# InternRobotics/InternNav

Measured on NVIDIA H100. Metric: InternVLA-N1 policy-steps/sec (batch RGB-D+text->action), higher is better.
Workload: dtype bf16

## Files before the change

### internnav_b200/csrc/attention_cache_wgmma.cu

```cuda
#include <math.h>

#include <mutex>

#include "dec_tile.cuh"

namespace n1 {
namespace {

constexpr int HD = 128, BKEY = 64, kStages = 4;
constexpr int kHalf = BKEY * 128;
constexpr int kBlockBytes = 2 * kHalf;
constexpr int kStageBytes = 2 * kBlockBytes;
constexpr int kQBytes = 2 * 128 * 128;
constexpr int kConsumerWarps = 8;
constexpr int kThreads = 32 * kConsumerWarps + 32;
constexpr int kSmem = kStages * kStageBytes + kQBytes + 256 + 1024;
static_assert(kSmem <= 232448, "attention_cache: shared memory budget");

struct CacheArgs {
  const bf16 *k, *v;
  int ldkv;
  bf16* o;
  int ldo;
  const int *cu_q, *ctx, *row0;
// ... 114 lines not shown
      const int k0 = n * BKEY + quad * 2;
      float alpha[2], m_s[2];
#pragma unroll
      for (int h = 0; h < 2; ++h) {
        float m = mx[h];
#pragma unroll
        for (int j = 0; j < 8; ++j)
#pragma unroll
          for (int e = 0; e < 2; ++e)
            if (k0 + j * 8 + e < vis[h]) m = fmaxf(m, s[4 * j + 2 * h + e]);
        m = fmaxf(m, __shfl_xor_sync(0xffffffffu, m, 1));
        m = fmaxf(m, __shfl_xor_sync(0xffffffffu, m, 2));
        alpha[h] = fast_exp2((mx[h] - m) * a.scale_log2);
        mx[h] = m;
        m_s[h] = m * a.scale_log2;
        sum[h] *= alpha[h];
      }
#pragma unroll
      for (int j = 0; j < 16; ++j) {
        o[4 * j + 0] *= alpha[0], o[4 * j + 1] *= alpha[0];
        o[4 * j + 2] *= alpha[1], o[4 * j + 3] *= alpha[1];
      }
      uint32_t pa[4][4];
#pragma unroll
      for (int j = 0; j < 8; ++j)
#pragma unroll
        for (int h = 0; h < 2; ++h) {
          const int kk = k0 + j * 8;
          const float p0 = kk < vis[h] ? fast_exp2(s[4 * j + 2 * h] * a.scale_log2 - m_s[h]) : 0.f;
          const float p1 = kk + 1 < vis[h] ? fast_exp2(s[4 * j + 2 * h + 1] * a.scale_log2 - m_s[h]) : 0.f;
          sum[h] += p0 + p1;
          pa[j >> 1][(j & 1) * 2 + h] = pack_bf16(p0, p1);
        }
      wgmma_fence();
#pragma unroll
      for (int ks = 0; ks < 4; ++ks) {
        const uint64_t bd = wgmma_desc_sw128(smem_u32(sV + ks * 16 * 128), kHalf);
        wgmma_rs<1>(o, pa[ks], bd, 1u);
      }
      wgmma_commit();
      wgmma_wait<0>();
      __syncwarp();
      if (lane == 0) mbar_arrive(empty + st);
    }
#pragma unroll
    for (int h = 0; h < 2; ++h) {
      float l = sum[h];
      l += __shfl_xor_sync(0xffffffffu, l, 1);
      l += __shfl_xor_sync(0xffffffffu, l, 2);
      const float inv = l > 0.f ? 1.0f / l : 0.f;
      if (qrow[h] >= 0) {
        const int m = m_a + h * 8;
        bf16* orow = a.o + (long)(q_start + qrow[h]) * a.ldo + (kh * G + m % G) * HD + quad * 2;
#pragma unroll
        for (int j = 0; j < 16; ++j)
          *reinterpret_cast<uint32_t*>(orow + j * 8) = pack_bf16(o[4 * j + 2 * h] * inv, o[4 * j + 2 * h + 1] * inv);
      }
    }
  }
}

}

void attention_cache(const CacheAttnParams& p, cudaStream_t stream) {
  if (p.batch <= 0) return;
  N1_CHECK(p.heads_kv > 0 && p.heads_q % p.heads_kv == 0 && p.heads_q / p.heads_kv <= 64,
           "attention_cache: heads_q must be a multiple of heads_kv (at most 64 per group)");
  N1_CHECK(p.ldq % 8 == 0 && p.ldkv % 8 == 0 && p.ldo % 8 == 0 && p.max_chunk > 0 && p.q_rows > 0 && p.kv_rows > 0,
           "attention_cache: bad strides / sizes");
  N1_CHECK((reinterpret_cast<uintptr_t>(p.k) & 15) == 0 && (reinterpret_cast<uintptr_t>(p.v) & 15) == 0 &&
               (reinterpret_cast<uintptr_t>(p.o) & 15) == 0,
           "attention_cache: 16-byte alignment");
  N1_CHECK(p.batch <= 65535 && p.heads_kv <= 65535, "attention_cache: grid too large");
  static std::once_flag once;
  std::call_once(once, [] { cudaFuncSetAttribute(attn_cache_kernel, cudaFuncAttributeMaxDynamicSharedMemorySize, kSmem); });
  CacheArgs a;
  a.k = p.k, a.v = p.v, a.ldkv = p.ldkv, a.o = p.o, a.ldo = p.ldo;
  a.cu_q = p.cu_q, a.ctx = p.ctx, a.row0 = p.row0;
  a.group = p.heads_q / p.heads_kv;
  a.rows_wg = 64 / a.group;
  a.scale_log2 = p.scale * 1.4426950408889634f;
  const long qd[3] = {HD, p.heads_q, p.q_rows}, qs[2] = {HD, p.ldq};
  const int qb[3] = {64, a.group, a.rows_wg};
  CUtensorMap tmQ = tma_map_3d_sw128(p.q, qd, qs, qb);
  CUtensorMap tmK = tma_map_2d(p.k, p.kv_rows, (long)p.heads_kv * HD, p.ldkv, BKEY, 64, true);
  CUtensorMap tmV = tma_map_2d(p.v, p.kv_rows, (long)p.heads_kv * HD, p.ldkv, BKEY, 64, true);
  const int tiles = (p.max_chunk + 2 * a.rows_wg - 1) / (2 * a.rows_wg);
  dim3 grid(tiles, p.heads_kv, p.batch);
  attn_cache_kernel<<<grid, kThreads, kSmem, stream>>>(tmQ, tmK, tmV, a);
  prof_count_launch();
  N1_CUDA(cudaGetLastError());
}

}
```

### internnav_b200/csrc/dec_attn_block.cu

```cuda
#include <mutex>

#include "dec_tile.cuh"

namespace n1 {
namespace {

constexpr int D = 384, HD = 48, BM = 64;
constexpr int kABytes = BM * D * 2;
constexpr int kSlots = 2, kSlotBytes = D * 64 * 2;
constexpr int kKvRow = 112;
constexpr int kKvBytes = BM * kKvRow;
constexpr int kConsumerWarps = 8;
constexpr int kThreads = 32 * kConsumerWarps + 128;
constexpr int kSmem = 2 * kABytes + kSlots * kSlotBytes + 2 * 2 * kKvBytes + 256 + 1024;
static_assert(kSmem <= 232448, "dec_attn_block: shared memory budget (227 KB per block)");

struct DecAttnArgs {
  bf16* x;
  int ldx;
  const float* ln_w;
  const float* ln_b;
  float eps;
  const float* b_in;
  const float* b_o;
  const bf16* kv;
  int ldkv;
  int mtok;
  int Ns, T, tpt, tiles_per_env, tiles;
  int causal;
};

__device__ __forceinline__ void warpgroup_barrier(int g) { asm volatile("bar.sync %0, 128;" ::"r"(2 + g) : "memory"); }

template <bool kSelf>
__global__ void __launch_bounds__(kThreads, 1)
dec_attn_kernel(const __grid_constant__ CUtensorMap tmIn, const __grid_constant__ CUtensorMap tmO, const DecAttnArgs args) {
  constexpr int NP = kSelf ? 3 * HD : HD;
  constexpr int kHeadBytes = NP * 64 * 2;
  extern __shared__ uint8_t smem_raw[];
  uint8_t* smem = reinterpret_cast<uint8_t*>((reinterpret_cast<uintptr_t>(smem_raw) + 1023) & ~uintptr_t(1023));
  uint8_t* sA = smem;
  uint8_t* sO = smem + kABytes;
  uint8_t* sW = sO + kABytes;
  uint8_t* sKV = sW + kSlots * kSlotBytes;
  uint64_t* bars = reinterpret_cast<uint64_t*>(sKV + 4 * kKvBytes);
  uint64_t* full = bars;
  uint64_t* empty = bars + kSlots;

  const int warp = threadIdx.x >> 5, lane = threadIdx.x & 31;
  if (threadIdx.x == 0) {
    tma_prefetch_desc(&tmIn), tma_prefetch_desc(&tmO);
    for (int s = 0; s < kSlots; ++s) mbar_init(&full[s], 1), mbar_init(&empty[s], kConsumerWarps);
    fence_mbar_init();
  }
  __syncthreads();

  if (warp >= kConsumerWarps) {
    setmaxnreg_dec<kProducerRegs>();
    if (warp == kConsumerWarps && lane == 0) {
      Ring<kSlots> r;
      for (int t = blockIdx.x; t < args.tiles; t += gridDim.x) {
        for (int hp = 0; hp < 4; ++hp)
          for (int kb = 0; kb < D / 64; ++kb) {
            mbar_wait(&empty[r.slot], r.phase ^ 1);
            mbar_arrive_expect_tx(&full[r.slot], 2 * kHeadBytes);
            uint8_t* dst = sW + r.slot * kSlotBytes;
#pragma unroll
            for (int g = 0; g < 2; ++g) {
              const int h = 4 * g + hp;
#pragma unroll
              for (int part = 0; part < NP / HD; ++part)
                tma_load_2d(dst + g * kHeadBytes + part * HD * 128, &tmIn, &full[r.slot], kb * 64, part * D + h * HD);
            }
            r.advance();
          }
        for (int kb = 0; kb < D / 64; ++kb) {
          mbar_wait(&empty[r.slot], r.phase ^ 1);
          mbar_arrive_expect_tx(&full[r.slot], kSlotBytes);
          uint8_t* dst = sW + r.slot * kSlotBytes;
          tma_load_2d(dst, &tmO, &full[r.slot], kb * 64, 0);
          tma_load_2d(dst + kSlotBytes / 2, &tmO, &full[r.slot], kb * 64, 192);
          r.advance();
        }
      }
    }
  } else {
    setmaxnreg_inc<kConsumerRegs>();
    const int cw = warp;
    const int g = cw >> 2;
    const int wtid = threadIdx.x & 127;
    const int quad = lane & 3;
    const int r0 = (cw & 3) * 16 + (lane >> 2);
    uint8_t* sK = sKV + g * 2 * kKvBytes;
    uint8_t* sV = sK + kKvBytes;
    const float sl2 = 0.14433756729740643f * 1.4426950408889634f;
    Ring<kSlots> ring;
    for (int t = blockIdx.x; t < args.tiles; t += gridDim.x) {
      const int env = t / args.tiles_per_env;
      const int traj0 = (t - env * args.tiles_per_env) * args.tpt;
      const int ntraj = min(args.tpt, args.Ns - traj0);
      const long row0 = ((long)env * args.Ns + traj0) * args.T;
      const int nrows = ntraj * args.T;
      consumer_barrier();
      ln384_to_tile<false>(sA, args.x, args.ldx, row0, nrows, args.ln_w, args.ln_b, args.eps, cw, lane);
      fence_proxy_async_smem();
      consumer_barrier();

      for (int hp = 0; hp < 4; ++hp) {
        const int h = 4 * g + hp;
        warpgroup_barrier(g);
        if (!kSelf) {
          const bf16* kb0 = args.kv + (long)env * args.mtok * args.ldkv + h * HD;
          for (int c = wtid; c < 2 * BM * 6; c += 128) {
            const int v = c / (BM * 6), j = (c / 6) % BM, ch = c % 6;
            uint4 val = make_uint4(0u, 0u, 0u, 0u);
            if (j < args.mtok) val = __ldg(reinterpret_cast<const uint4*>(kb0 + (long)j * args.ldkv + v * D + ch * 8));
            *reinterpret_cast<uint4*>((v ? sV : sK) + j * kKvRow + ch * 16) = val;
          }
        }
        float acc[NP / 2];
        mma_k384(acc, sA, sW, full, empty, ring, kSlotBytes, g * kHeadBytes, lane, [] {});
        uint32_t qf[3][4];
#pragma unroll
        for (int j = 0; j < NP / 8; ++j) {
          const int part = j / 6, c = (j % 6) * 8 + quad * 2;
          const float2 b = __ldg(reinterpret_cast<const float2*>(args.b_in + part * D + h * HD + c));
          const uint32_t lo = pack_bf16(acc[4 * j] + b.x, acc[4 * j + 1] + b.y);
          const uint32_t hi = pack_bf16(acc[4 * j + 2] + b.x, acc[4 * j + 3] + b.y);
          if (part == 0) {
            qf[j >> 1][(j & 1) * 2] = lo, qf[j >> 1][(j & 1) * 2 + 1] = hi;
          } else {
            uint8_t* buf = part == 1 ? sK : sV;
            *reinterpret_cast<uint32_t*>(buf + r0 * kKvRow + c * 2) = lo;
            *reinterpret_cast<uint32_t*>(buf + (r0 + 8) * kKvRow + c * 2) = hi;
          }
        }
        warpgroup_barrier(g);
        int lo_key[2], hi_key[2];
#pragma unroll
        for (int r = 0; r < 2; ++r) {
          const int qi = r0 + 8 * r;
          if (kSelf) {
            lo_key[r] = qi / args.T * args.T;
            hi_key[r] = args.causal ? qi : lo_key[r] + args.T - 1;
          } else {
            lo_key[r] = 0, hi_key[r] = args.mtok - 1;
          }
        }
        float o[6][4], inv0, inv1;
        attn_hd48_16rows<4>(qf, sK, sV, kKvRow, lo_key, hi_key, sl2, lane, o, inv0, inv1);
#pragma unroll
        for (int i = 0; i < 6; ++i) {
          const int col = h * HD + i * 8 + quad * 2;
          *reinterpret_cast<uint32_t*>(sO + sw128_offset(r0, col)) = pack_bf16(o[i][0] * inv0, o[i][1] * inv0);
          *reinterpret_cast<uint32_t*>(sO + sw128_offset(r0 + 8, col)) = pack_bf16(o[i][2] * inv1, o[i][3] * inv1);
        }
      }
      fence_proxy_async_smem();
      consumer_barrier();
      float y[96] = {};
      mma_k384(y, sO, sW, full, empty, ring, kSlotBytes, g * (kSlotBytes / 2), lane, [] {});
      residual_epilogue_192<false>(y, args.x, args.ldx, args.x, args.ldx, args.b_o, row0, nrows, g, r0, quad);
    }
  }
}

template <bool kSelf>
void launch_dec_attn(const bf16* w_in, const bf16* w_o, const DecAttnArgs& a, long rows, cudaStream_t stream) {
  static std::once_flag once;
  std::call_once(once, [] { cudaFuncSetAttribute(dec_attn_kernel<kSelf>, cudaFuncAttributeMaxDynamicSharedMemorySize, kSmem); });
  const CUtensorMap tmIn = tma_map_2d(w_in, kSelf ? 3 * D : D, D, D, HD, 64, true);
  const CUtensorMap tmO = tma_map_2d(w_o, D, D, D, 192, 64, true);
  const int sms = device_sm_count();
  const int grid = a.tiles < sms ? a.tiles : sms;
  const int N = kSelf ? 4 * D : 2 * D;
  const double flops = 2.0 * rows * (double)N * D;
  const int ticket = prof_begin(flops, (int)rows, N, D, stream);
  dec_attn_kernel<kSelf><<<grid, kThreads, kSmem, stream>>>(tmIn, tmO, a);
  prof_end(ticket, stream);
  prof_count_gemm(flops);
  N1_CUDA(cudaGetLastError());
}

DecAttnArgs dec_args(bf16* x, int ldx, const float* ln_w, const float* ln_b, float eps, const float* b_in, const float* b_o,
                     int B, int Ns, int T) {
  N1_CHECK(x && ln_w && ln_b && b_in && b_o, "dec_attn_block: null pointer");
  N1_CHECK((reinterpret_cast<uintptr_t>(x) & 15) == 0 && ldx % 8 == 0 && ldx >= D, "dec_attn_block: misaligned x");
  N1_CHECK(B >= 1 && Ns >= 1 && T >= 1 && T <= BM, "dec_attn_block: needs B, Ns >= 1 and 1 <= T <= 64");
  DecAttnArgs a = {};
  a.x = x, a.ldx = ldx, a.ln_w = ln_w, a.ln_b = ln_b, a.eps = eps, a.b_in = b_in, a.b_o = b_o;
  a.Ns = Ns, a.T = T, a.tpt = BM / T;
  a.tiles_per_env = (Ns + a.tpt - 1) / a.tpt;
  const long tiles = (long)B * a.tiles_per_env;
  N1_CHECK(tiles < (1L << 31), "dec_attn_block: too many tiles");
  a.tiles = (int)tiles;
  return a;
}

}

void dec_sa_block(bf16* x, int ldx, const float* ln_w, const float* ln_b, float eps, const bf16* w_qkv, const float* b_qkv,
                  const bf16* w_o, const float* b_o, int B, int Ns, int T, int causal, cudaStream_t stream) {
  N1_CHECK(w_qkv && w_o, "dec_sa_block: null weights");
  DecAttnArgs a = dec_args(x, ldx, ln_w, ln_b, eps, b_qkv, b_o, B, Ns, T);
  a.causal = causal ? 1 : 0;
  launch_dec_attn<true>(w_qkv, w_o, a, (long)B * Ns * T, stream);
}

void dec_ca_block(bf16* x, int ldx, const float* ln_w, const float* ln_b, float eps, const bf16* w_q, const float* b_q,
                  const bf16* w_o, const float* b_o, const bf16* kv, int ldkv, int mtok, int B, int Ns, int T,
                  cudaStream_t stream) {
  N1_CHECK(w_q && w_o && kv, "dec_ca_block: null weights or K / V");
  N1_CHECK(mtok >= 1 && mtok <= BM, "dec_ca_block: needs 1 <= condition tokens <= 64");
  N1_CHECK((reinterpret_cast<uintptr_t>(kv) & 15) == 0 && ldkv % 8 == 0 && ldkv >= 2 * D, "dec_ca_block: misaligned K / V");
  DecAttnArgs a = dec_args(x, ldx, ln_w, ln_b, eps, b_q, b_o, B, Ns, T);
  a.kv = kv, a.ldkv = ldkv, a.mtok = mtok;
  launch_dec_attn<false>(w_q, w_o, a, (long)B * Ns * T, stream);
}

}
```

### internnav_b200/csrc/dec_tile.cuh

```cuda
#pragma once
#include "n1_ops.h"
#include "n1_ptx.cuh"

namespace n1 {

__device__ __forceinline__ int sw128_offset(int row, int col) {
  return (col >> 6) * 8192 + (row >> 3) * 1024 + (row & 7) * 128 + ((((col & 63) >> 3) ^ (row & 7)) << 4) + (col & 7) * 2;
}

template <int kS>
struct Ring {
  int slot = 0;
  uint32_t phase = 0;
  __device__ __forceinline__ void advance() {
    if (++slot == kS) slot = 0, phase ^= 1;
  }
};

template <bool kNc>
__device__ __forceinline__ void ln384_to_tile(uint8_t* sA, const bf16* x, long ldx, long row0, int nrows, const float* ln_w,
                                              const float* ln_b, float eps, int cw, int lane) {
  constexpr int D = 384;
  uint2 q[8][3];
#pragma unroll
  for (int rr = 0; rr < 8; ++rr) {
    const int r = cw * 8 + rr;
    const uint2* xr = reinterpret_cast<const uint2*>(x + (row0 + r) * ldx);
#pragma unroll
    for (int i = 0; i < 3; ++i)
      q[rr][i] = r < nrows ? (kNc ? __ldg(xr + lane + i * 32) : xr[lane + i * 32]) : make_uint2(0u, 0u);
  }
  float s[8], sq[8];
#pragma unroll
  for (int rr = 0; rr < 8; ++rr) {
    s[rr] = 0.f;
#pragma unroll
    for (int i = 0; i < 3; ++i)
      s[rr] += bf16_lo(q[rr][i].x) + bf16_hi(q[rr][i].x) + bf16_lo(q[rr][i].y) + bf16_hi(q[rr][i].y);
  }
#pragma unroll
  for (int o = 16; o > 0; o >>= 1)
#pragma unroll
    for (int rr = 0; rr < 8; ++rr) s[rr] += __shfl_xor_sync(0xffffffffu, s[rr], o);
#pragma unroll
  for (int rr = 0; rr < 8; ++rr) {
    const float mu = s[rr] * (1.0f / D);
    s[rr] = mu;
    sq[rr] = 0.f;
#pragma unroll
    for (int i = 0; i < 3; ++i) {
      const float a = bf16_lo(q[rr][i].x) - mu, b = bf16_hi(q[rr][i].x) - mu;
      const float c = bf16_lo(q[rr][i].y) - mu, d = bf16_hi(q[rr][i].y) - mu;
      sq[rr] += a * a + b * b + c * c + d * d;
    }
  }
#pragma unroll
  for (int o = 16; o > 0; o >>= 1)
#pragma unroll
    for (int rr = 0; rr < 8; ++rr) sq[rr] += __shfl_xor_sync(0xffffffffu, sq[rr], o);
#pragma unroll
  for (int i = 0; i < 3; ++i) {
    const int col = (lane + i * 32) * 4;
    const float4 lw = __ldg(reinterpret_cast<const float4*>(ln_w + col));
    const float4 lb = __ldg(reinterpret_cast<const float4*>(ln_b + col));
#pragma unroll
    for (int rr = 0; rr < 8; ++rr) {
      const float mu = s[rr], rstd = rsqrtf(sq[rr] * (1.0f / D) + eps);
      const float y0 = (bf16_lo(q[rr][i].x) - mu) * rstd * lw.x + lb.x, y1 = (bf16_hi(q[rr][i].x) - mu) * rstd * lw.y + lb.y;
      const float y2 = (bf16_lo(q[rr][i].y) - mu) * rstd * lw.z + lb.z, y3 = (bf16_hi(q[rr][i].y) - mu) * rstd * lw.w + lb.w;
      *reinterpret_cast<uint2*>(sA + sw128_offset(cw * 8 + rr, col)) = make_uint2(pack_bf16(y0, y1), pack_bf16(y2, y3));
    }
  }
}

template <int N, int kS, typename AfterFirst>
__device__ __forceinline__ void mma_k384(float (&acc)[N], const uint8_t* sA, const uint8_t* ring, uint64_t* full,
                                         uint64_t* empty, Ring<kS>& rs, int slot_bytes, int b_offset, int lane,
                                         AfterFirst after_first) {
  int prev = -1;
#pragma unroll 1
  for (int kb = 0; kb < 6; ++kb) {
    mbar_wait(&full[rs.slot], rs.phase);
    const uint64_t ad = wgmma_desc_sw128(smem_u32(sA + kb * 8192));
    const uint64_t bd = wgmma_desc_sw128(smem_u32(ring + rs.slot * slot_bytes + b_offset));
    wgmma_fence();
#pragma unroll
    for (int k = 0; k < 4; ++k) wgmma_ss<0, 0>(acc, ad + 2 * k, bd + 2 * k, (kb | k) != 0 ? 1u : 0u);
    wgmma_commit();
    wgmma_wait<1>();
    if (kb == 0) after_first();
    if (lane == 0 && prev >= 0) mbar_arrive(&empty[prev]);
    prev = rs.slot;
    rs.advance();
  }
  wgmma_wait<0>();
  if (lane == 0) mbar_arrive(&empty[prev]);
}

template <bool kNc>
__device__ __forceinline__ void residual_epilogue_192(const float (&y)[96], const bf16* x, long ldx, bf16* out, long ldo,
                                                      const float* bias, long row0, int nrows, int g, int r0, int quad) {
#pragma unroll
  for (int hh = 0; hh < 2; ++hh) {
    const int r = r0 + hh * 8;
    if (r >= nrows) continue;
    const bf16* xr = x + (row0 + r) * ldx + g * 192 + quad * 2;
    bf16* orow = out + (row0 + r) * ldo + g * 192 + quad * 2;
#pragma unroll
    for (int jj = 0; jj < 24; ++jj) {
      const uint32_t* xp = reinterpret_cast<const uint32_t*>(xr + jj * 8);
      const uint32_t xv = kNc ? __ldg(xp) : *xp;
      const float2 b = __ldg(reinterpret_cast<const float2*>(bias + g * 192 + jj * 8 + quad * 2));
      *reinterpret_cast<uint32_t*>(orow + jj * 8) =
          pack_bf16(y[jj * 4 + 2 * hh] + bf16_lo(xv) + b.x, y[jj * 4 + 2 * hh + 1] + bf16_hi(xv) + b.y);
    }
  }
}

template <int NKP>
__device__ __forceinline__ void attn_hd48_16rows(const uint32_t (&qf)[3][4], const uint8_t* sK, const uint8_t* sV,
                                                 int row_bytes, const int (&lo_key)[2], const int (&hi_key)[2], float sl2,
                                                 int lane, float (&o)[6][4], float& inv0, float& inv1) {
  const int lm = lane >> 3, lr = lane & 7;
  float s[2 * NKP][4];
#pragma unroll
  for (int i = 0; i < 2 * NKP; ++i) s[i][0] = s[i][1] = s[i][2] = s[i][3] = 0.f;
#pragma unroll
  for (int ks = 0; ks < 3; ++ks)
#pragma unroll
    for (int np = 0; np < NKP; ++np) {
      uint32_t b0, b1, b2, b3;
      ldsm_x4(smem_u32(sK + (np * 16 + (lm >> 1) * 8 + lr) * row_bytes + (ks * 16 + (lm & 1) * 8) * 2), b0, b1, b2, b3);
      mma_bf16(s[2 * np], qf[ks], b0, b1);
      mma_bf16(s[2 * np + 1], qf[ks], b2, b3);
    }
  float mx[2] = {-INFINITY, -INFINITY};
#pragma unroll
  for (int i = 0; i < 2 * NKP; ++i)
#pragma unroll
    for (int e = 0; e < 4; ++e) {
      const int key = i * 8 + (lane & 3) * 2 + (e & 1), r = e >> 1;
      const bool vis = key >= lo_key[r] && key <= hi_key[r];
      s[i][e] = vis ? s[i][e] * sl2 : -INFINITY;
      mx[r] = fmaxf(mx[r], s[i][e]);
    }
  float sum[2] = {0.f, 0.f};
#pragma unroll
  for (int r = 0; r < 2; ++r) {
    mx[r] = fmaxf(mx[r], __shfl_xor_sync(0xffffffffu, mx[r], 1));
    mx[r] = fmaxf(mx[r], __shfl_xor_sync(0xffffffffu, mx[r], 2));
    if (mx[r] == -INFINITY) mx[r] = 0.f;
  }
  uint32_t pf[NKP][4];
#pragma unroll
  for (int i = 0; i < 2 * NKP; ++i) {
    const float p0 = exp2f(s[i][0] - mx[0]), p1 = exp2f(s[i][1] - mx[0]);
    const float p2 = exp2f(s[i][2] - mx[1]), p3 = exp2f(s[i][3] - mx[1]);
    sum[0] += p0 + p1, sum[1] += p2 + p3;
    pf[i >> 1][(i & 1) * 2 + 0] = pack_bf16(p0, p1);
    pf[i >> 1][(i & 1) * 2 + 1] = pack_bf16(p2, p3);
  }
#pragma unroll
  for (int r = 0; r < 2; ++r) {
    sum[r] += __shfl_xor_sync(0xffffffffu, sum[r], 1);
    sum[r] += __shfl_xor_sync(0xffffffffu, sum[r], 2);
  }
#pragma unroll
  for (int i = 0; i < 6; ++i) o[i][0] = o[i][1] = o[i][2] = o[i][3] = 0.f;
#pragma unroll
  for (int kk = 0; kk < NKP; ++kk)
#pragma unroll
    for (int np = 0; np < 3; ++np) {
      uint32_t b0, b1, b2, b3;
      ldsm_x4_t(smem_u32(sV + (kk * 16 + (lm & 1) * 8 + lr) * row_bytes + (np * 16 + (lm >> 1) * 8) * 2), b0, b1, b2, b3);
      mma_bf16(o[2 * np], pf[kk], b0, b1);
      mma_bf16(o[2 * np + 1], pf[kk], b2, b3);
    }
  inv0 = sum[0] > 0.f ? 1.f / sum[0] : 0.f;
  inv1 = sum[1] > 0.f ? 1.f / sum[1] : 0.f;
}

}
```

### internnav_b200/csrc/gemm_wgmma.cu

```cuda
#include <stdlib.h>

#include <algorithm>
#include <atomic>
#include <mutex>
#include <vector>

#include "n1_ops.h"
#include "n1_ptx.cuh"

namespace n1 {

namespace {

constexpr int BM = 128;
constexpr int BK = 64;
constexpr int kConsumerWarps = 8;
constexpr int kThreads = 32 * kConsumerWarps + 128;

template <int BN>
struct Cfg {
  static constexpr int kABytes = BM * BK * 2;
  static constexpr int kBBytes = BN * BK * 2;
  static constexpr int kStageBytes = kABytes + kBBytes;
  static constexpr int kStages = BN == 256 ? 4 : BN == 128 ? 6 : 8;
// ... 294 lines not shown
  cuuint64_t gdim[2] = {(cuuint64_t)cols, (cuuint64_t)rows};
  cuuint64_t gstr[1] = {(cuuint64_t)ld * 2};
  cuuint32_t box[2] = {(cuuint32_t)box_cols, (cuuint32_t)box_rows};
  cuuint32_t estr[2] = {1, 1};
  CUresult r = encode_fn()(&m, CU_TENSOR_MAP_DATA_TYPE_BFLOAT16, 2, const_cast<bf16*>(ptr), gdim, gstr, box, estr,
                           CU_TENSOR_MAP_INTERLEAVE_NONE, swizzle, CU_TENSOR_MAP_L2_PROMOTION_L2_256B,
                           CU_TENSOR_MAP_FLOAT_OOB_FILL_NONE);
  if (r != CUDA_SUCCESS) throw Error(-5, "cuTensorMapEncodeTiled failed: " + std::to_string((int)r));
  return m;
}

template <int BN, int KIND>
constexpr auto kernel_of() {
  if constexpr (KIND == KIND_LINEAR_SWIGLU) return gemm_kernel<BN>;
  else return gemm_act_kernel<BN, KIND>;
}

template <int BN, int KIND>
void launch(const bf16* A, int lda, const bf16* W, int ldw, int M, int N, int K, GemmArgs& a, cudaStream_t stream) {
  using C = Cfg<BN>;
  auto* kernel = kernel_of<BN, KIND>();
  static std::once_flag once;
  std::call_once(once, [kernel] {
    cudaFuncSetAttribute(kernel, cudaFuncAttributeMaxDynamicSharedMemorySize, C::kSmemBytes);
  });
  a.tiles_m = (M + BM - 1) / BM;
  a.tiles_n = (N + BN - 1) / BN;
  {
    const long panel = (long)BM * K * 2;
    const long w_bytes = (long)N * K * 2;
    int g = 8;
    if (w_bytes > kWStreamsBytes) g = (int)std::max<long>(2, (16L << 20) / panel);
    a.raster_g = g < a.tiles_m ? g : a.tiles_m;
    if (a.raster_g < 1) a.raster_g = 1;
  }
  CUtensorMap tmA = make_map(A, M, K, lda, BM);
  CUtensorMap tmB = make_map(W, N, K, ldw, BN);
  CUtensorMap tmC = tmA;
  if (KIND != KIND_GENERAL) {
    const bool sw = a.act == ACT_SWIGLU;
    tmC = make_map(static_cast<const bf16*>(a.out), M, sw ? N / 2 : N, a.ldo, 16, sw ? 16 : 32,
                   sw ? CU_TENSOR_MAP_SWIZZLE_32B : CU_TENSOR_MAP_SWIZZLE_64B);
  }
  const int tiles = a.tiles_m * a.tiles_n;
  const int grid = tiles < device_sm_count() ? tiles : device_sm_count();
  kernel<<<grid, kThreads, C::kSmemBytes, stream>>>(tmA, tmB, tmC, a);
  N1_CUDA(cudaGetLastError());
}

template <int BN>
void launch_kind(int kind, const bf16* A, int lda, const bf16* W, int ldw, int M, int N, int K, GemmArgs& a,
                 cudaStream_t stream) {
  switch (kind) {
    case KIND_LINEAR_SWIGLU: return launch<BN, KIND_LINEAR_SWIGLU>(A, lda, W, ldw, M, N, K, a, stream);
    case ACT_GELU: return launch<BN, ACT_GELU>(A, lda, W, ldw, M, N, K, a, stream);
    case ACT_RELU: return launch<BN, ACT_RELU>(A, lda, W, ldw, M, N, K, a, stream);
    case ACT_GELU_TANH: return launch<BN, ACT_GELU_TANH>(A, lda, W, ldw, M, N, K, a, stream);
    case ACT_SILU: return launch<BN, ACT_SILU>(A, lda, W, ldw, M, N, K, a, stream);
    default: return launch<BN, KIND_GENERAL>(A, lda, W, ldw, M, N, K, a, stream);
  }
}

std::atomic<long> g_total_launches{0}, g_gemm_launches{0};
std::atomic<bool> g_prof_on{false};
std::mutex g_prof_mu;
struct EvPair {
  cudaEvent_t a, b;
  double flops;
  int M, N, K;
};
std::vector<EvPair> g_events;
struct ShapeAcc {
  int M, N, K;
  long count;
  double ms;
};
std::vector<ShapeAcc> g_shapes;

}

CUtensorMap tma_map_2d(const bf16* ptr, long rows, long cols, long ld, int box_rows, int box_cols, bool swizzle) {
  return make_map(ptr, rows, cols, ld, box_rows, box_cols, swizzle ? CU_TENSOR_MAP_SWIZZLE_128B : CU_TENSOR_MAP_SWIZZLE_NONE);
}
CUtensorMap tma_map_3d_sw128(const bf16* ptr, const long dims[3], const long strides[2], const int box[3]) {
  N1_CHECK((reinterpret_cast<uintptr_t>(ptr) & 15) == 0 && strides[0] % 8 == 0 && strides[1] % 8 == 0,
           "tma_map_3d_sw128: 16-byte alignment");
  CUtensorMap m;
  cuuint64_t gdim[3] = {(cuuint64_t)dims[0], (cuuint64_t)dims[1], (cuuint64_t)dims[2]};
  cuuint64_t gstr[2] = {(cuuint64_t)strides[0] * 2, (cuuint64_t)strides[1] * 2};
  cuuint32_t bx[3] = {(cuuint32_t)box[0], (cuuint32_t)box[1], (cuuint32_t)box[2]};
  cuuint32_t estr[3] = {1, 1, 1};
  CUresult r = encode_fn()(&m, CU_TENSOR_MAP_DATA_TYPE_BFLOAT16, 3, const_cast<bf16*>(ptr), gdim, gstr, bx, estr,
                           CU_TENSOR_MAP_INTERLEAVE_NONE, CU_TENSOR_MAP_SWIZZLE_128B, CU_TENSOR_MAP_L2_PROMOTION_L2_256B,
                           CU_TENSOR_MAP_FLOAT_OOB_FILL_NONE);
  if (r != CUDA_SUCCESS) throw Error(-5, "cuTensorMapEncodeTiled (3-D) failed: " + std::to_string((int)r));
  return m;
}
void prof_count_gemm(double flops) {
  (void)flops;
  g_gemm_launches++;
  g_total_launches++;
}

void prof_enable(bool on) { g_prof_on = on; }
int prof_begin(double flops, int M, int N, int K, cudaStream_t s) {
  if (!g_prof_on.load()) return -1;
  EvPair ev{};
  cudaEventCreate(&ev.a);
  cudaEventCreate(&ev.b);
  ev.flops = flops, ev.M = M, ev.N = N, ev.K = K;
  cudaEventRecord(ev.a, s);
  std::lock_guard<std::mutex> lk(g_prof_mu);
  g_events.push_back(ev);
  return (int)g_events.size() - 1;
}
void prof_end(int ticket, cudaStream_t s) {
  if (ticket < 0) return;
  std::lock_guard<std::mutex> lk(g_prof_mu);
  if (ticket < (int)g_events.size()) cudaEventRecord(g_events[ticket].b, s);
}
void prof_count_launch(int n) { g_total_launches += n; }
ProfStats prof_read_and_reset() {
  ProfStats st;
  std::lock_guard<std::mutex> lk(g_prof_mu);
  for (EvPair& e : g_events) {
    cudaEventSynchronize(e.b);
    float ms = 0.f;
    if (cudaEventElapsedTime(&ms, e.a, e.b) == cudaSuccess) {
      st.gemm_ms += ms, st.gemm_flops += e.flops;
      bool hit = false;
      for (ShapeAcc& sa : g_shapes)
        if (sa.M == e.M && sa.N == e.N && sa.K == e.K) {
          sa.count++, sa.ms += ms, hit = true;
          break;
        }
      if (!hit) g_shapes.push_back({e.M, e.N, e.K, 1, (double)ms});
    }
    cudaEventDestroy(e.a);
    cudaEventDestroy(e.b);
  }
  g_events.clear();
  st.gemm_launches = g_gemm_launches.exchange(0);
  st.total_launches = g_total_launches.exchange(0);
  return st;
}

int prof_read_shapes(int* mnk, long* count, double* ms, int cap) {
  std::lock_guard<std::mutex> lk(g_prof_mu);
  int n = 0;
  for (const ShapeAcc& sa : g_shapes) {
    if (n >= cap) break;
    mnk[3 * n] = sa.M, mnk[3 * n + 1] = sa.N, mnk[3 * n + 2] = sa.K;
    count[n] = sa.count, ms[n] = sa.ms;
    ++n;
  }
  g_shapes.clear();
  return n;
}

int device_sm_count() {
  static int sms = 0;
  if (!sms) {
    int dev = 0;
    cudaGetDevice(&dev);
    cudaDeviceGetAttribute(&sms, cudaDevAttrMultiProcessorCount, dev);
    if (sms <= 0) sms = 132;
  }
  return sms;
}

void gemm_bf16(const bf16* A, int lda, const bf16* W, int ldw, void* out, int ldo, int M, int N, int K,
               const GemmEpilogue& e, cudaStream_t stream, int tile_n) {
  if (M <= 0 || N <= 0) return;
  N1_CHECK(tile_n == 0 || tile_n == 64 || tile_n == 128 || tile_n == 256, "GEMM tile width must be 0, 64, 128 or 256");
  N1_CHECK(K > 0 && K % 8 == 0, "GEMM K must be a positive multiple of 8");
  N1_CHECK(N % 8 == 0, "GEMM N must be a multiple of 8 (pad the packed weight)");
  N1_CHECK(!(e.act == ACT_SWIGLU) || N % 16 == 0, "SwiGLU GEMM needs N % 16 == 0");
// ... 37 lines not shown
```

### internnav_b200/csrc/n1_ops.h

```cpp
#pragma once
#include <cuda.h>
#include <cuda_bf16.h>
#include <cuda_runtime.h>
#include <stdint.h>

#include <stdexcept>
#include <string>

namespace n1 {

typedef __nv_bfloat16 bf16;

struct Error : std::runtime_error {
  int code;
  Error(int c, const std::string& m) : std::runtime_error(m), code(c) {}
};

#define N1_CHECK(cond, msg)                                                                       \
  do {                                                                                            \
    if (!(cond)) throw ::n1::Error(-2, std::string(__FILE__) + ":" + std::to_string(__LINE__) + \
                                           ": " + (msg));                                         \
  } while (0)

#define N1_CUDA(call)                                                                              \
  do {                                                                                             \
    cudaError_t e__ = (call);                                                                      \
    if (e__ != cudaSuccess)                                                                        \
      throw ::n1::Error(-3, std::string(__FILE__) + ":" + std::to_string(__LINE__) + ": " + #call + \
                                ": " + cudaGetErrorString(e__));                                   \
  } while (0)

enum GemmAct { ACT_NONE = 0, ACT_GELU = 1, ACT_RELU = 2, ACT_SWIGLU = 3, ACT_GELU_TANH = 4, ACT_SILU = 5 };

struct GemmEpilogue {
  const float* bias = nullptr;
  const float* gamma = nullptr;
  const bf16* residual = nullptr;
  int ldr = 0;
  int act = ACT_NONE;
  int out_fp32 = 0;
  int rows_per_group = 0, group_stride = 0, group_offset = 0;
  const float* row_add = nullptr;
};

void gemm_bf16(const bf16* A, int lda, const bf16* W, int ldw, void* out, int ldo, int M, int N, int K,
               const GemmEpilogue& epi, cudaStream_t stream, int tile_n = 0);

int device_sm_count();

CUtensorMap tma_map_2d(const bf16* ptr, long rows, long cols, long ld, int box_rows, int box_cols, bool swizzle);
CUtensorMap tma_map_3d_sw128(const bf16* ptr, const long dims[3], const long strides[2], const int box[3]);
void prof_count_gemm(double flops);

struct ProfStats {
  double gemm_ms = 0, gemm_flops = 0;
  long gemm_launches = 0, total_launches = 0;
};
void prof_enable(bool on);
void prof_count_launch(int n = 1);
int prof_begin(double flops, int M, int N, int K, cudaStream_t s);
void prof_end(int ticket, cudaStream_t s);
ProfStats prof_read_and_reset();
int prof_read_shapes(int* mnk, long* count, double* ms, int cap);

void layernorm(const bf16* x, int ldx, bf16* y, int ldy, const float* w, const float* b, int rows, int D,
               float eps, int rms, cudaStream_t stream);

struct AttnParams {
  const bf16* q;
  const bf16* k;
  const bf16* v;
  bf16* o;
  int ldq, ldk, ldv, ldo;
  int heads_q, heads_kv, hd;
  int batch;
  int seq_q, seq_k;
  const int* cu_q;
  const int* cu_k;
  int kv_div;
  int causal;
  float scale;
  int max_seq_q;
  const int* k_len;
  int k_slot;
  long total_rows;
  const int* k_row0;
};
void attention(const AttnParams& p, cudaStream_t stream);
bool attention_tc_supported(const AttnParams& p);
bool attention_uses_tc(const AttnParams& p);
void attention_tc128(const AttnParams& p, cudaStream_t stream);

struct CacheAttnParams {
  const bf16* q;
  int ldq;
  long q_rows;
  const bf16 *k, *v;
  int ldkv;
  long kv_rows;
  bf16* o;
  int ldo;
  const int *cu_q, *ctx, *row0;
  int batch, max_chunk, heads_q, heads_kv;
  float scale;
};
void attention_cache(const CacheAttnParams& p, cudaStream_t stream);

void ff_block_384(const bf16* x, int ldx, const float* ln_w, const float* ln_b, float eps, const bf16* w1, const float* b1,
                  const bf16* w2, const float* b2, bf16* out, int ldo, int M, cudaStream_t stream);
void dec_sa_block(bf16* x, int ldx, const float* ln_w, const float* ln_b, float eps, const bf16* w_qkv, const float* b_qkv,
                  const bf16* w_o, const float* b_o, int B, int Ns, int T, int causal, cudaStream_t stream);
void dec_ca_block(bf16* x, int ldx, const float* ln_w, const float* ln_b, float eps, const bf16* w_q, const float* b_q,
                  const bf16* w_o, const float* b_o, const bf16* kv, int ldkv, int mtok, int B, int Ns, int T,
                  cudaStream_t stream);

void mod_norm(const bf16* x, int ldx, const float* w, const bf16* mod, int ld_mod, int rows_per_group, const bf16* res, int ldr,
              bf16* out, int ldo, long rows, int D, float eps, int mode, cudaStream_t stream);
void add_bf16(const bf16* a, const bf16* b, bf16* out, long n, cudaStream_t stream);
void action_embed(const float* lat, const float* w, const float* b, const float* pos, bf16* out, long rows, int T, int D,
                  cudaStream_t stream);
void cfg_euler(const bf16* pred, int ld, long n, int cfg, float scale, float dt, float* lat, cudaStream_t stream);

void traj_to_actions(const float* traj, int B, int Ns, int T, double turn_rad, double step_size, int lookahead,
                     int max_actions, int cap, int* ids, int* count, double* mean_out, cudaStream_t s);
void traj_mean_path(const float* traj, int B, int Ns, int T, double* mean_out, cudaStream_t s);

}
```

Measured before the change: 71.17.

## Overlap decoder attention with projections and TMA-load cross-attention K/V

The self-attention path now runs the attention for the previous head pair inside the next head's QKV projection mainloop, through a hook moved to after the slot release. The cross-attention path computes all four query heads in one wide GEMM and streams K/V per head pair by TMA into spare buffers, replacing the per-warpgroup __ldg copies. The shared attention helper also skips key blocks that lie outside each warp's visible range. Together these are meant to hide memory latency and drop wasted MMA work, at the cost of more complex barrier phase tracking and reuse of the A buffer for K/V.

```diff
diff --git a/internnav_b200/csrc/attention_cache_wgmma.cu b/internnav_b200/csrc/attention_cache_wgmma.cu
--- a/internnav_b200/csrc/attention_cache_wgmma.cu
+++ b/internnav_b200/csrc/attention_cache_wgmma.cu
@@ -220,7 +220,7 @@
   a.scale_log2 = p.scale * 1.4426950408889634f;
   const long qd[3] = {HD, p.heads_q, p.q_rows}, qs[2] = {HD, p.ldq};
   const int qb[3] = {64, a.group, a.rows_wg};
-  CUtensorMap tmQ = tma_map_3d_sw128(p.q, qd, qs, qb);
+  CUtensorMap tmQ = tma_map_3d(p.q, qd, qs, qb, true);
   CUtensorMap tmK = tma_map_2d(p.k, p.kv_rows, (long)p.heads_kv * HD, p.ldkv, BKEY, 64, true);
   CUtensorMap tmV = tma_map_2d(p.v, p.kv_rows, (long)p.heads_kv * HD, p.ldkv, BKEY, 64, true);
   const int tiles = (p.max_chunk + 2 * a.rows_wg - 1) / (2 * a.rows_wg);
diff --git a/internnav_b200/csrc/dec_attn_block.cu b/internnav_b200/csrc/dec_attn_block.cu
--- a/internnav_b200/csrc/dec_attn_block.cu
+++ b/internnav_b200/csrc/dec_attn_block.cu
@@ -10,10 +10,13 @@
 constexpr int kSlots = 2, kSlotBytes = D * 64 * 2;
 constexpr int kKvRow = 112;
 constexpr int kKvBytes = BM * kKvRow;
+constexpr int kCaHead = BM * HD * 2;
+constexpr int kCaStep = 2 * 2 * kCaHead;
 constexpr int kConsumerWarps = 8;
 constexpr int kThreads = 32 * kConsumerWarps + 128;
 constexpr int kSmem = 2 * kABytes + kSlots * kSlotBytes + 2 * 2 * kKvBytes + 256 + 1024;
 static_assert(kSmem <= 232448, "dec_attn_block: shared memory budget (227 KB per block)");
+static_assert(kCaStep <= 2 * 2 * kKvBytes && 2 * kCaStep == kABytes, "dec_attn_block: cross K / V buffers");
 
 struct DecAttnArgs {
   bf16* x;
@@ -34,9 +37,10 @@
 
 template <bool kSelf>
 __global__ void __launch_bounds__(kThreads, 1)
-dec_attn_kernel(const __grid_constant__ CUtensorMap tmIn, const __grid_constant__ CUtensorMap tmO, const DecAttnArgs args) {
-  constexpr int NP = kSelf ? 3 * HD : HD;
-  constexpr int kHeadBytes = NP * 64 * 2;
+dec_attn_kernel(const __grid_constant__ CUtensorMap tmIn, const __grid_constant__ CUtensorMap tmO,
+                const __grid_constant__ CUtensorMap tmKV, const DecAttnArgs args) {
+  constexpr int kHeadBytes = 3 * HD * 64 * 2;
+  constexpr int kInFills = kSelf ? 24 : 6;
   extern __shared__ uint8_t smem_raw[];
   uint8_t* smem = reinterpret_cast<uint8_t*>((reinterpret_cast<uintptr_t>(smem_raw) + 1023) & ~uintptr_t(1023));
   uint8_t* sA = smem;
@@ -46,11 +50,16 @@
   uint64_t* bars = reinterpret_cast<uint64_t*>(sKV + 4 * kKvBytes);
   uint64_t* full = bars;
   uint64_t* empty = bars + kSlots;
+  uint64_t* kv_full = bars + 2 * kSlots;
+  uint64_t* kv_free = kv_full + 4;
 
   const int warp = threadIdx.x >> 5, lane = threadIdx.x & 31;
   if (threadIdx.x == 0) {
     tma_prefetch_desc(&tmIn), tma_prefetch_desc(&tmO);
+    if (!kSelf) tma_prefetch_desc(&tmKV);
     for (int s = 0; s < kSlots; ++s) mbar_init(&full[s], 1), mbar_init(&empty[s], kConsumerWarps);
+    for (int s = 0; s < 4; ++s) mbar_init(&kv_full[s], 1);
+    mbar_init(kv_free, kConsumerWarps);
     fence_mbar_init();
   }
   __syncthreads();
@@ -59,28 +68,46 @@
     setmaxnreg_dec<kProducerRegs>();
     if (warp == kConsumerWarps && lane == 0) {
       Ring<kSlots> r;
+      uint32_t free_phase = 0;
+      auto load_kv = [&](int hp, int env, uint8_t* dst) {
+        mbar_arrive_expect_tx(&kv_full[hp], kCaStep);
+#pragma unroll
+        for (int g = 0; g < 2; ++g) {
+          const int h = 4 * g + hp;
+          tma_load_3d(dst + g * 2 * kCaHead, &tmKV, &kv_full[hp], h * HD, 0, env);
+          tma_load_3d(dst + g * 2 * kCaHead + kCaHead, &tmKV, &kv_full[hp], D + h * HD, 0, env);
+        }
+      };
       for (int t = blockIdx.x; t < args.tiles; t += gridDim.x) {
-        for (int hp = 0; hp < 4; ++hp)
-          for (int kb = 0; kb < D / 64; ++kb) {
-            mbar_wait(&empty[r.slot], r.phase ^ 1);
+        const int env = t / args.tiles_per_env;
+        if (!kSelf) {
+          mbar_wait(kv_free, free_phase ^ 1), free_phase ^= 1;
+          load_kv(0, env, sKV);
+        }
+        for (int i = 0; i < kInFills + D / 64; ++i) {
+          mbar_wait(&empty[r.slot], r.phase ^ 1);
+          if (!kSelf && i == kInFills + 1) load_kv(1, env, sA), load_kv(2, env, sA + kCaStep);
+          uint8_t* dst = sW + r.slot * kSlotBytes;
+          if (kSelf && i < kInFills) {
+            const int hp = i / 6, kb = i % 6;
             mbar_arrive_expect_tx(&full[r.slot], 2 * kHeadBytes);
-            uint8_t* dst = sW + r.slot * kSlotBytes;
-#pragma unroll
-            for (int g = 0; g < 2; ++g) {
-              const int h = 4 * g + hp;
-#pragma unroll
-              for (int part = 0; part < NP / HD; ++part)
-                tma_load_2d(dst + g * kHeadBytes + part * HD * 128, &tmIn, &full[r.slot], kb * 64, part * D + h * HD);
-            }
-            r.advance();
-          }
-        for (int kb = 0; kb < D / 64; ++kb) {
-          mbar_wait(&empty[r.slot], r.phase ^ 1);
-          mbar_arrive_expect_tx(&full[r.slot], kSlotBytes);
-          uint8_t* dst = sW + r.slot * kSlotBytes;
-          tma_load_2d(dst, &tmO, &full[r.slot], kb * 64, 0);
-          tma_load_2d(dst + kSlotBytes / 2, &tmO, &full[r.slot], kb * 64, 192);
+#pragma unroll
+            for (int g = 0; g < 2; ++g)
+#pragma unroll
+              for (int part = 0; part < 3; ++part)
+                tma_load_2d(dst + g * kHeadBytes + part * HD * 128, &tmIn, &full[r.slot], kb * 64, part * D + (4 * g + hp) * HD);
+          } else {
+            const CUtensorMap* m = i < kInFills ? &tmIn : &tmO;
+            const int kb = i < kInFills ? i : i - kInFills;
+            mbar_arrive_expect_tx(&full[r.slot], kSlotBytes);
+            tma_load_2d(dst, m, &full[r.slot], kb * 64, 0);
+            tma_load_2d(dst + kSlotBytes / 2, m, &full[r.slot], kb * 64, 192);
+          }
           r.advance();
+          if (!kSelf && i == kInFills + 1) {
+            mbar_wait(kv_free, free_phase ^ 1), free_phase ^= 1;
+            load_kv(3, env, sKV);
+          }
         }
       }
     }
@@ -88,13 +115,21 @@
     setmaxnreg_inc<kConsumerRegs>();
     const int cw = warp;
     const int g = cw >> 2;
-    const int wtid = threadIdx.x & 127;
     const int quad = lane & 3;
     const int r0 = (cw & 3) * 16 + (lane >> 2);
     uint8_t* sK = sKV + g * 2 * kKvBytes;
     uint8_t* sV = sK + kKvBytes;
     const float sl2 = 0.14433756729740643f * 1.4426950408889634f;
     Ring<kSlots> ring;
+    uint32_t kv_phase = 0;
+    auto store_o = [&](int h, const float (&o)[6][4], float inv0, float inv1) {
+#pragma unroll
+      for (int i = 0; i < 6; ++i) {
+        const int col = h * HD + i * 8 + quad * 2;
+        *reinterpret_cast<uint32_t*>(sO + sw128_offset(r0, col)) = pack_bf16(o[i][0] * inv0, o[i][1] * inv0);
+        *reinterpret_cast<uint32_t*>(sO + sw128_offset(r0 + 8, col)) = pack_bf16(o[i][2] * inv1, o[i][3] * inv1);
+      }
+    };
     for (int t = blockIdx.x; t < args.tiles; t += gridDim.x) {
       const int env = t / args.tiles_per_env;
       const int traj0 = (t - env * args.tiles_per_env) * args.tpt;
@@ -106,55 +141,69 @@
       fence_proxy_async_smem();
       consumer_barrier();
 
-      for (int hp = 0; hp < 4; ++hp) {
-        const int h = 4 * g + hp;
-        warpgroup_barrier(g);
-        if (!kSelf) {
-          const bf16* kb0 = args.kv + (long)env * args.mtok * args.ldkv + h * HD;
-          for (int c = wtid; c < 2 * BM * 6; c += 128) {
-            const int v = c / (BM * 6), j = (c / 6) % BM, ch = c % 6;
-            uint4 val = make_uint4(0u, 0u, 0u, 0u);
-            if (j < args.mtok) val = __ldg(reinterpret_cast<const uint4*>(kb0 + (long)j * args.ldkv + v * D + ch * 8));
-            *reinterpret_cast<uint4*>((v ? sV : sK) + j * kKvRow + ch * 16) = val;
-          }
-        }
-        float acc[NP / 2];
-        mma_k384(acc, sA, sW, full, empty, ring, kSlotBytes, g * kHeadBytes, lane, [] {});
+      if (kSelf) {
         uint32_t qf[3][4];
-#pragma unroll
-        for (int j = 0; j < NP / 8; ++j) {
-          const int part = j / 6, c = (j % 6) * 8 + quad * 2;
-          const float2 b = __ldg(reinterpret_cast<const float2*>(args.b_in + part * D + h * HD + c));
-          const uint32_t lo = pack_bf16(acc[4 * j] + b.x, acc[4 * j + 1] + b.y);
-          const uint32_t hi = pack_bf16(acc[4 * j + 2] + b.x, acc[4 * j + 3] + b.y);
-          if (part == 0) {
-            qf[j >> 1][(j & 1) * 2] = lo, qf[j >> 1][(j & 1) * 2 + 1] = hi;
-          } else {
-            uint8_t* buf = part == 1 ? sK : sV;
-            *reinterpret_cast<uint32_t*>(buf + r0 * kKvRow + c * 2) = lo;
-            *reinterpret_cast<uint32_t*>(buf + (r0 + 8) * kKvRow + c * 2) = hi;
-          }
-        }
-        warpgroup_barrier(g);
-        int lo_key[2], hi_key[2];
-#pragma unroll
-        for (int r = 0; r < 2; ++r) {
-          const int qi = r0 + 8 * r;
-          if (kSelf) {
+        auto attend = [&](int hp) {
+          int lo_key[2], hi_key[2];
+#pragma unroll
+          for (int r = 0; r < 2; ++r) {
+            const int qi = r0 + 8 * r;
             lo_key[r] = qi / args.T * args.T;
             hi_key[r] = args.causal ? qi : lo_key[r] + args.T - 1;
-          } else {
-            lo_key[r] = 0, hi_key[r] = args.mtok - 1;
-          }
-        }
-        float o[6][4], inv0, inv1;
-        attn_hd48_16rows<4>(qf, sK, sV, kKvRow, lo_key, hi_key, sl2, lane, o, inv0, inv1);
-#pragma unroll
-        for (int i = 0; i < 6; ++i) {
-          const int col = h * HD + i * 8 + quad * 2;
-          *reinterpret_cast<uint32_t*>(sO + sw128_offset(r0, col)) = pack_bf16(o[i][0] * inv0, o[i][1] * inv0);
-          *reinterpret_cast<uint32_t*>(sO + sw128_offset(r0 + 8, col)) = pack_bf16(o[i][2] * inv1, o[i][3] * inv1);
-        }
+          }
+          float o[6][4], inv0, inv1;
+          attn_hd48_16rows<4>(qf, sK, sV, kKvRow, lo_key, hi_key, sl2, lane, o, inv0, inv1);
+          store_o(4 * g + hp, o, inv0, inv1);
+        };
+        for (int hp = 0; hp < 4; ++hp) {
+          const int h = 4 * g + hp;
+          float acc[3 * HD / 2] = {};
+          mma_k384(acc, sA, sW, full, empty, ring, kSlotBytes, g * kHeadBytes, lane, [&] { if (hp > 0) attend(hp - 1); }, 1);
+          warpgroup_barrier(g);
+#pragma unroll
+          for (int j = 0; j < 3 * HD / 8; ++j) {
+            const int part = j / 6, c = (j % 6) * 8 + quad * 2;
+            const float2 b = __ldg(reinterpret_cast<const float2*>(args.b_in + part * D + h * HD + c));
+            const uint32_t lo = pack_bf16(acc[4 * j] + b.x, acc[4 * j + 1] + b.y);
+            const uint32_t hi = pack_bf16(acc[4 * j + 2] + b.x, acc[4 * j + 3] + b.y);
+            if (part == 0) {
+              qf[j >> 1][(j & 1) * 2] = lo, qf[j >> 1][(j & 1) * 2 + 1] = hi;
+            } else {
+              uint8_t* buf = part == 1 ? sK : sV;
+              *reinterpret_cast<uint32_t*>(buf + r0 * kKvRow + c * 2) = lo;
+              *reinterpret_cast<uint32_t*>(buf + (r0 + 8) * kKvRow + c * 2) = hi;
+            }
+          }
+          warpgroup_barrier(g);
+        }
+        attend(3);
+      } else {
+        uint32_t qf[4][3][4];
+        {
+          float acc[96] = {};
+          mma_k384(acc, sA, sW, full, empty, ring, kSlotBytes, g * (kSlotBytes / 2), lane, [] {});
+#pragma unroll
+          for (int j = 0; j < 24; ++j) {
+            const int hp = j / 6, jj = j % 6;
+            const float2 b = __ldg(reinterpret_cast<const float2*>(args.b_in + g * 192 + j * 8 + quad * 2));
+            qf[hp][jj >> 1][(jj & 1) * 2] = pack_bf16(acc[4 * j] + b.x, acc[4 * j + 1] + b.y);
+            qf[hp][jj >> 1][(jj & 1) * 2 + 1] = pack_bf16(acc[4 * j + 2] + b.x, acc[4 * j + 3] + b.y);
+          }
+        }
+        const int lo_key[2] = {0, 0}, hi_key[2] = {args.mtok - 1, args.mtok - 1};
+#pragma unroll
+        for (int hp = 0; hp < 4; ++hp) {
+          mbar_wait(&kv_full[hp], kv_phase);
+          const uint8_t* k = (hp == 0 || hp == 3 ? sKV : sA + (hp - 1) * kCaStep) + g * 2 * kCaHead;
+          float o[6][4], inv0, inv1;
+          attn_hd48_16rows<4>(qf[hp], k, k + kCaHead, HD * 2, lo_key, hi_key, sl2, lane, o, inv0, inv1);
+          if (hp == 0 || hp == 3) {
+            __syncwarp();
+            if (lane == 0) mbar_arrive(kv_free);
+          }
+          store_o(4 * g + hp, o, inv0, inv1);
+        }
+        kv_phase ^= 1;
       }
       fence_proxy_async_smem();
       consumer_barrier();
@@ -169,14 +218,21 @@
 void launch_dec_attn(const bf16* w_in, const bf16* w_o, const DecAttnArgs& a, long rows, cudaStream_t stream) {
   static std::once_flag once;
   std::call_once(once, [] { cudaFuncSetAttribute(dec_attn_kernel<kSelf>, cudaFuncAttributeMaxDynamicSharedMemorySize, kSmem); });
-  const CUtensorMap tmIn = tma_map_2d(w_in, kSelf ? 3 * D : D, D, D, HD, 64, true);
+  const CUtensorMap tmIn = tma_map_2d(w_in, kSelf ? 3 * D : D, D, D, kSelf ? HD : 192, 64, true);
   const CUtensorMap tmO = tma_map_2d(w_o, D, D, D, 192, 64, true);
+  CUtensorMap tmKV = tmO;
+  if (!kSelf) {
+    const long dims[3] = {2 * D, a.mtok, a.tiles / a.tiles_per_env};
+    const long strides[2] = {a.ldkv, (long)a.mtok * a.ldkv};
+    const int box[3] = {HD, BM, 1};
+    tmKV = tma_map_3d(a.kv, dims, strides, box, false);
+  }
   const int sms = device_sm_count();
   const int grid = a.tiles < sms ? a.tiles : sms;
   const int N = kSelf ? 4 * D : 2 * D;
   const double flops = 2.0 * rows * (double)N * D;
   const int ticket = prof_begin(flops, (int)rows, N, D, stream);
-  dec_attn_kernel<kSelf><<<grid, kThreads, kSmem, stream>>>(tmIn, tmO, a);
+  dec_attn_kernel<kSelf><<<grid, kThreads, kSmem, stream>>>(tmIn, tmO, tmKV, a);
   prof_end(ticket, stream);
   prof_count_gemm(flops);
   N1_CUDA(cudaGetLastError());
diff --git a/internnav_b200/csrc/dec_tile.cuh b/internnav_b200/csrc/dec_tile.cuh
--- a/internnav_b200/csrc/dec_tile.cuh
+++ b/internnav_b200/csrc/dec_tile.cuh
@@ -73,10 +73,10 @@
   }
 }
 
-template <int N, int kS, typename AfterFirst>
+template <int N, int kS, typename Hook>
 __device__ __forceinline__ void mma_k384(float (&acc)[N], const uint8_t* sA, const uint8_t* ring, uint64_t* full,
-                                         uint64_t* empty, Ring<kS>& rs, int slot_bytes, int b_offset, int lane,
-                                         AfterFirst after_first) {
+                                         uint64_t* empty, Ring<kS>& rs, int slot_bytes, int b_offset, int lane, Hook hook,
+                                         int hook_kb = 0) {
   int prev = -1;
 #pragma unroll 1
   for (int kb = 0; kb < 6; ++kb) {
@@ -88,8 +88,8 @@
     for (int k = 0; k < 4; ++k) wgmma_ss<0, 0>(acc, ad + 2 * k, bd + 2 * k, (kb | k) != 0 ? 1u : 0u);
     wgmma_commit();
     wgmma_wait<1>();
-    if (kb == 0) after_first();
     if (lane == 0 && prev >= 0) mbar_arrive(&empty[prev]);
+    if (kb == hook_kb) hook();
     prev = rs.slot;
     rs.advance();
   }
@@ -122,6 +122,8 @@
                                                  int row_bytes, const int (&lo_key)[2], const int (&hi_key)[2], float sl2,
                                                  int lane, float (&o)[6][4], float& inv0, float& inv1) {
   const int lm = lane >> 3, lr = lane & 7;
+  const int kb_lo = __reduce_min_sync(0xffffffffu, min(lo_key[0], lo_key[1])) >> 4;
+  const int kb_hi = __reduce_max_sync(0xffffffffu, max(hi_key[0], hi_key[1])) >> 4;
   float s[2 * NKP][4];
 #pragma unroll
   for (int i = 0; i < 2 * NKP; ++i) s[i][0] = s[i][1] = s[i][2] = s[i][3] = 0.f;
@@ -129,6 +131,7 @@
   for (int ks = 0; ks < 3; ++ks)
 #pragma unroll
     for (int np = 0; np < NKP; ++np) {
+      if (np < kb_lo || np > kb_hi) continue;
       uint32_t b0, b1, b2, b3;
       ldsm_x4(smem_u32(sK + (np * 16 + (lm >> 1) * 8 + lr) * row_bytes + (ks * 16 + (lm & 1) * 8) * 2), b0, b1, b2, b3);
       mma_bf16(s[2 * np], qf[ks], b0, b1);
@@ -154,6 +157,7 @@
   uint32_t pf[NKP][4];
 #pragma unroll
   for (int i = 0; i < 2 * NKP; ++i) {
+    if ((i >> 1) < kb_lo || (i >> 1) > kb_hi) continue;
     const float p0 = exp2f(s[i][0] - mx[0]), p1 = exp2f(s[i][1] - mx[0]);
     const float p2 = exp2f(s[i][2] - mx[1]), p3 = exp2f(s[i][3] - mx[1]);
     sum[0] += p0 + p1, sum[1] += p2 + p3;
@@ -171,6 +175,7 @@
   for (int kk = 0; kk < NKP; ++kk)
 #pragma unroll
     for (int np = 0; np < 3; ++np) {
+      if (kk < kb_lo || kk > kb_hi) continue;
       uint32_t b0, b1, b2, b3;
       ldsm_x4_t(smem_u32(sV + (kk * 16 + (lm & 1) * 8 + lr) * row_bytes + (np * 16 + (lm >> 1) * 8) * 2), b0, b1, b2, b3);
       mma_bf16(o[2 * np], pf[kk], b0, b1);
diff --git a/internnav_b200/csrc/gemm_wgmma.cu b/internnav_b200/csrc/gemm_wgmma.cu
--- a/internnav_b200/csrc/gemm_wgmma.cu
+++ b/internnav_b200/csrc/gemm_wgmma.cu
@@ -400,17 +400,17 @@
 CUtensorMap tma_map_2d(const bf16* ptr, long rows, long cols, long ld, int box_rows, int box_cols, bool swizzle) {
   return make_map(ptr, rows, cols, ld, box_rows, box_cols, swizzle ? CU_TENSOR_MAP_SWIZZLE_128B : CU_TENSOR_MAP_SWIZZLE_NONE);
 }
-CUtensorMap tma_map_3d_sw128(const bf16* ptr, const long dims[3], const long strides[2], const int box[3]) {
+CUtensorMap tma_map_3d(const bf16* ptr, const long dims[3], const long strides[2], const int box[3], bool swizzle) {
   N1_CHECK((reinterpret_cast<uintptr_t>(ptr) & 15) == 0 && strides[0] % 8 == 0 && strides[1] % 8 == 0,
-           "tma_map_3d_sw128: 16-byte alignment");
+           "tma_map_3d: 16-byte alignment");
   CUtensorMap m;
   cuuint64_t gdim[3] = {(cuuint64_t)dims[0], (cuuint64_t)dims[1], (cuuint64_t)dims[2]};
   cuuint64_t gstr[2] = {(cuuint64_t)strides[0] * 2, (cuuint64_t)strides[1] * 2};
   cuuint32_t bx[3] = {(cuuint32_t)box[0], (cuuint32_t)box[1], (cuuint32_t)box[2]};
   cuuint32_t estr[3] = {1, 1, 1};
   CUresult r = encode_fn()(&m, CU_TENSOR_MAP_DATA_TYPE_BFLOAT16, 3, const_cast<bf16*>(ptr), gdim, gstr, bx, estr,
-                           CU_TENSOR_MAP_INTERLEAVE_NONE, CU_TENSOR_MAP_SWIZZLE_128B, CU_TENSOR_MAP_L2_PROMOTION_L2_256B,
-                           CU_TENSOR_MAP_FLOAT_OOB_FILL_NONE);
+                           CU_TENSOR_MAP_INTERLEAVE_NONE, swizzle ? CU_TENSOR_MAP_SWIZZLE_128B : CU_TENSOR_MAP_SWIZZLE_NONE,
+                           CU_TENSOR_MAP_L2_PROMOTION_L2_256B, CU_TENSOR_MAP_FLOAT_OOB_FILL_NONE);
   if (r != CUDA_SUCCESS) throw Error(-5, "cuTensorMapEncodeTiled (3-D) failed: " + std::to_string((int)r));
   return m;
 }
diff --git a/internnav_b200/csrc/n1_ops.h b/internnav_b200/csrc/n1_ops.h
--- a/internnav_b200/csrc/n1_ops.h
+++ b/internnav_b200/csrc/n1_ops.h
@@ -49,7 +49,7 @@
 int device_sm_count();
 
 CUtensorMap tma_map_2d(const bf16* ptr, long rows, long cols, long ld, int box_rows, int box_cols, bool swizzle);
-CUtensorMap tma_map_3d_sw128(const bf16* ptr, const long dims[3], const long strides[2], const int box[3]);
+CUtensorMap tma_map_3d(const bf16* ptr, const long dims[3], const long strides[2], const int box[3], bool swizzle);
 void prof_count_gemm(double flops);
 
 struct ProfStats {
```

Result: no change. 71.85, median of 6 (+1.0%).
